# zhanxinrui/HDN

Measured on AMD Instinct MI355X. Metric: frames/sec on 127/255 template/search pairs, higher is better.
Workload: dtype f32; 1 GPU; BASELINE configs[1]: batch=64 synthetic 127/255 pairs per GPU, 256-ch features; HIP kernels only: 1x xcorr 31x31(x)61x61 + 6x xcorr 5x5(x)29x29 + 6x circular xcorr 13x13(x)13x13 + 3x PreShareFeature 127x127 + fused DLT/warp + the 2 L1 scores (one launch); pairs_per_gpu=64, channels=256

## Files before the change

hdn_amd/csrc/xcorr.hip:

```cpp
#include <atomic>

#include "hdn_common.h"
#include "circ13_tables.h"

#include <type_traits>

#include <cstdlib>

#define HDN_ABL_XCORR_0(...) __VA_ARGS__
#define HDN_ABL_XCORR_1(...) __VA_ARGS__
#ifdef HDN_ABLATION
#include "ablation/xcorr.inc"
#endif

namespace hdn {

constexpr int XC_MAX_PROBLEMS = 8;

struct XcorrPtrs {
  const float* x[XC_MAX_PROBLEMS];
  const float* k[XC_MAX_PROBLEMS];
  float* out[XC_MAX_PROBLEMS];
};

namespace prod29 {
constexpr int HX = 29, WX = 29, HK = 5, WK = 5, HO = 25, WO = 25;
constexpr int XPLANE = HX * WX, OPLANE = HO * WO, KPLANE = HK * WK;
constexpr int SX = 37, LPLANE = HX * SX;
constexpr int PPB = 4;
constexpr int UNITS = 5 * WO;
constexpr int XFLOATS = round_up(PPB * LPLANE + 8, 4);
#ifndef PROD29_ALIAS
#define PROD29_ALIAS 0
#endif
#ifndef PROD29_PAD_FLOATS
#define PROD29_PAD_FLOATS 0
#endif
constexpr int LDS_FLOATS = (PROD29_ALIAS ? XFLOATS : XFLOATS + PPB * OPLANE) + PROD29_PAD_FLOATS;
constexpr int N4 = PPB * XPLANE / 4;
constexpr int ITER = cdiv(N4, HDN_BLOCK);
}

__global__ __launch_bounds__(HDN_BLOCK) void xcorr_prod29_kernel(XcorrPtrs P, int planes) {
  using namespace prod29;
  HDN_ABL_XCORR_0()
  __shared__ __attribute__((aligned(16))) float smem[LDS_FLOATS];
  float* sx = smem;
  float* so = PROD29_ALIAS ? smem : smem + XFLOATS;

  const int tid = threadIdx.x;
  const int lane = tid & (HDN_WAVE - 1);
  const int wave = __builtin_amdgcn_readfirstlane(tid >> 6);
  const int prob = blockIdx.y;
  const float* __restrict__ x = P.x[prob];
  const float* __restrict__ k = P.k[prob];
  float* __restrict__ out = P.out[prob];
  const int plane0 = blockIdx.x * PPB;
  const int np = min(PPB, planes - plane0);
  const float* xg = x + size_t(plane0) * XPLANE;

  if (np == PPB && aligned16(xg)) {
    const float4* s4 = reinterpret_cast<const float4*>(xg);
    float4 r[ITER];
#pragma unroll
    for (int q = 0; q < ITER; ++q) r[q] = ld_stream(s4 + min(tid + q * HDN_BLOCK, N4 - 1));
#pragma unroll
    for (int q = 0; q < ITER; ++q) {
      const int i4 = tid + q * HDN_BLOCK;
      if (i4 < N4) {
        const float v[4] = {r[q].x, r[q].y, r[q].z, r[q].w};
        const int e0 = 4 * i4, row0 = e0 / WX, c0 = e0 - row0 * WX;
        if (c0 + 3 < WX) {
          *reinterpret_cast<float4*>(sx + e0 + (SX - WX) * row0) = r[q];
        } else {
#pragma unroll
          for (int t = 0; t < 4; ++t) sx[e0 + t + (SX - WX) * (row0 + (c0 + t >= WX ? 1 : 0))] = v[t];
        }
      }
    }
  } else {
    for (int e = tid; e < np * XPLANE; e += HDN_BLOCK) {
      const int p = e / XPLANE, rem = e - p * XPLANE;
      const int rr = rem / WX, c = rem - rr * WX;
      sx[p * LPLANE + rr * SX + c] = xg[e];
    }
  }
  __syncthreads();

  float held[2][5];
  if (wave < np) {
    const float* __restrict__ kp = k + size_t(plane0 + wave) * KPLANE;
    const float* xs = sx + wave * LPLANE;
    float* os = so + wave * OPLANE;
#pragma unroll
    for (int rd = 0; rd < 2; ++rd) {
      const int unit = rd * HDN_WAVE + lane;
      const int uu = min(unit, UNITS - 1);
      const int b = uu / WO, j = uu - b * WO;
      const float* xc = xs + (5 * b) * SX + j;
      float acc[5] = {0.f, 0.f, 0.f, 0.f, 0.f};
#pragma unroll
      for (int v = 0; v < WK; ++v) {
        float col[9];
#pragma unroll
        for (int r = 0; r < 9; ++r) col[r] = xc[r * SX + v];
#pragma unroll
        for (int u = 0; u < HK; ++u) {
          const float kv = kp[u * WK + v];
#pragma unroll
          for (int t = 0; t < 5; ++t) acc[t] = __builtin_fmaf(col[t + u], kv, acc[t]);
        }
      }
      if constexpr (PROD29_ALIAS) {
#pragma unroll
        for (int t = 0; t < 5; ++t) held[rd][t] = acc[t];
      } else if (unit < UNITS) {
#pragma unroll
        for (int t = 0; t < 5; ++t) os[(5 * b + t) * WO + j] = acc[t];
      }
    }
  }
  __syncthreads();
  if constexpr (PROD29_ALIAS) {
    if (wave < np) {
      float* os = so + wave * OPLANE;
#pragma unroll
      for (int rd = 0; rd < 2; ++rd) {
        const int unit = rd * HDN_WAVE + lane;
        if (unit < UNITS) {
          const int b = unit / WO, j = unit - b * WO;
#pragma unroll
          for (int t = 0; t < 5; ++t) os[(5 * b + t) * WO + j] = held[rd][t];
        }
      }
    }
    __syncthreads();
  }

  float* og = out + size_t(plane0) * OPLANE;
  if (np == PPB && aligned16(og)) copy_l2g_full<PPB * OPLANE>(so, og, tid);
  else copy_l2g(so, og, np * OPLANE, tid);
}

namespace cfg5 {
constexpr int HX = 35, WX = 35, HK = 5, WK = 5, HO = 31, WO = 31;
constexpr int XPLANE = HX * WX, OPLANE = HO * WO, KPLANE = HK * WK;
constexpr int PPB = 4, TH = 8;
constexpr int XFLOATS = round_up(PPB * XPLANE + WX + 4, 4);
constexpr int LDS_FLOATS = XFLOATS + PPB * OPLANE;

typedef const float __attribute__((address_space(4))) cfloat;
template <int V, int M>
__device__ __forceinline__ void strip_pairs(float2v (&Pm)[6], uint32_t a0, uint32_t a1) {
  if constexpr (M < 6) {
    if constexpr (M < 3) Pm[M] = lds_read_pair<(2 * M) * WX + V, (2 * M + 1) * WX + V>(a0);
    else Pm[M] = lds_read_pair<(2 * M - 6) * WX + V, (2 * M - 5) * WX + V>(a1);
    strip_pairs<V, M + 1>(Pm, a0, a1);
  }
}
template <int V>
__device__ __forceinline__ void strip_column(float2v (&accE)[4], float2v (&accO)[5], uint32_t a0, uint32_t a1, const cfloat* kp) {
  float2v Pm[6];
  strip_pairs<V, 0>(Pm, a0, a1);
  lds_wait_all();
#pragma unroll
  for (int m = 0; m < 6; ++m) pin(Pm[m]);
#pragma unroll
  for (int u = 0; u < HK; ++u) {
    const float kv = kp[u * WK + V];
    const float2v kk = {kv, kv};
    if (u % 2 == 0) {
#pragma unroll
      for (int q = 0; q < 4; ++q) accE[q] = __builtin_elementwise_fma(Pm[q + u / 2], kk, accE[q]);
    } else {
#pragma unroll
      for (int q = 0; q < 5; ++q) accO[q] = __builtin_elementwise_fma(Pm[q + u / 2], kk, accO[q]);
    }
  }
}
__device__ __forceinline__ void strip(float (&acc)[TH], const float* x00, const cfloat* kp) {
  float2v accE[4], accO[5];
#pragma unroll
  for (int q = 0; q < 4; ++q) accE[q] = float2v{0.f, 0.f};
#pragma unroll
  for (int q = 0; q < 5; ++q) accO[q] = float2v{0.f, 0.f};
  const uint32_t a0 = lds_addr(x00), a1 = a0 + 6 * WX * 4;
  strip_column<0>(accE, accO, a0, a1, kp);
  strip_column<1>(accE, accO, a0, a1, kp);
  strip_column<2>(accE, accO, a0, a1, kp);
  strip_column<3>(accE, accO, a0, a1, kp);
  strip_column<4>(accE, accO, a0, a1, kp);
#pragma unroll
  for (int q = 0; q < 4; ++q) {
    acc[2 * q] = accE[q].x + accO[q].y;
    acc[2 * q + 1] = accE[q].y + accO[q + 1].x;
  }
}
__device__ __forceinline__ const cfloat* scalar_ptr(const float* p) {
  uint64_t a = reinterpret_cast<uint64_t>(p);
  asm volatile("" : "+s"(a));
  return (const cfloat*)a;
}
}

__global__ __launch_bounds__(HDN_BLOCK) void xcorr_cfg5_kernel(XcorrPtrs P, int planes) {
  using namespace cfg5;
  __shared__ __attribute__((aligned(16))) float smem[XFLOATS];
  float* sx = smem;
  float* so = smem;

  const int tid = threadIdx.x;
  const int lane = tid & (HDN_WAVE - 1);
  const int wave = __builtin_amdgcn_readfirstlane(tid >> 6);
  const int prob = blockIdx.y;
  const float* __restrict__ x = P.x[prob];
  const float* __restrict__ k = P.k[prob];
  float* __restrict__ out = P.out[prob];
  const int plane0 = blockIdx.x * PPB;
  const int np = min(PPB, planes - plane0);
  const float* xg = x + size_t(plane0) * XPLANE;

  if (np == PPB && aligned16(xg)) copy_g2l_full<PPB * XPLANE>(xg, sx, tid);
  else copy_g2l(xg, sx, np * XPLANE, tid);
  if (tid < WX + 4) sx[PPB * XPLANE + tid] = 0.f;
  __syncthreads();

  float accs[2][TH];
  if (wave < np) {
    const cfloat* kp = scalar_ptr(k + size_t(plane0 + wave) * KPLANE);
    const float* xs = sx + wave * XPLANE;
    const int j = min(lane & 31, WO - 1);
#pragma unroll
    for (int rd = 0; rd < 2; ++rd) {
      const int b = 2 * rd + (lane >> 5);
      strip(accs[rd], xs + (TH * b) * WX + j, kp);
    }
  }
  __syncthreads();
  if (wave < np && (lane & 31) < WO) {
    float* os = so + wave * OPLANE;
    const int j = lane & 31;
#pragma unroll
    for (int rd = 0; rd < 2; ++rd) {
      const int b = 2 * rd + (lane >> 5);
#pragma unroll
      for (int t = 0; t < TH; ++t)
        if (TH * b + t < HO) os[(TH * b + t) * WO + j] = accs[rd][t];
    }
  }
  __syncthreads();

  float* og = out + size_t(plane0) * OPLANE;
  if (np == PPB && aligned16(og)) copy_l2g_full<PPB * OPLANE>(so, og, tid);
  else copy_l2g(so, og, np * OPLANE, tid);
}

namespace north {
constexpr int HX = 61, WX = 61, HK = 31, WK = 31, HO = 31, WO = 31;
constexpr int XPLANE = HX * WX;
constexpr int OPLANE = HO * WO;
constexpr int SX = 68;
constexpr int NQUAD = 12;
constexpr int NQ = 15;
constexpr int WINDOW = NQ * HDN_WAVE * 4;
constexpr int GUARD_ROWS_BEFORE = 1, GUARD_ROWS_AFTER = 3;
constexpr int SLOT = (GUARD_ROWS_BEFORE + HX + GUARD_ROWS_AFTER) * SX;
constexpr size_t LDS_BYTES = size_t(4 * SLOT) * sizeof(float);

typedef float f16v __attribute__((ext_vector_type(16)));
typedef float f8v __attribute__((ext_vector_type(8)));
typedef float f4v __attribute__((ext_vector_type(4)));

struct Taps {
  f16v a;
  f8v b;
  f4v c;
  float2v d;
  float e;
  __device__ __forceinline__ float get(int v) const {
    return v < 16 ? a[v] : (v < 24 ? b[v - 16] : (v < 28 ? c[v - 24] : (v < 30 ? d[v - 28] : e)));
  }
};

struct Row {
  f4v Q[NQUAD];
  Taps k;
  __device__ __forceinline__ float2v pair(int n) const { return (n & 1) ? Q[n >> 1].zw : Q[n >> 1].xy; }
};

template <int M>
__device__ __forceinline__ void issue_quads(Row& R, uint32_t a) {
  if constexpr (M < NQUAD) {
    asm volatile("ds_read_b128 %0, %1 offset:%2" : "=v"(R.Q[M]) : "v"(a), "n"(M * 16));
    issue_quads<M + 1>(R, a);
  }
}

__device__ __forceinline__ void load_row(Row& R, uint32_t xaddr, const float* kr) {
  issue_quads<0>(R, xaddr);
  asm volatile(
      "s_nop 4\n\t"
      "s_load_dwordx16 %0, %5, 0x0\n\t"
      "s_load_dwordx8 %1, %5, 0x40\n\t"
      "s_load_dwordx4 %2, %5, 0x60\n\t"
      "s_load_dwordx2 %3, %5, 0x70\n\t"
      "s_load_dword %4, %5, 0x78"
      : "=&s"(R.k.a), "=&s"(R.k.b), "=&s"(R.k.c), "=&s"(R.k.d), "=&s"(R.k.e)
      : "s"(kr));
}

__device__ __forceinline__ void land_row(Row& R) {
  lds_wait_all();
#pragma unroll
  for (int m = 0; m < NQUAD; ++m) asm volatile("" : "+v"(R.Q[m]));
  asm volatile("" : "+s"(R.k.a), "+s"(R.k.b), "+s"(R.k.c), "+s"(R.k.d), "+s"(R.k.e));
  __builtin_amdgcn_sched_barrier(0);
}

__device__ __forceinline__ bool tap_nonzero(float kv) {
  unsigned b;
  asm("s_and_b32 %0, %1, 0x7fffffff" : "=s"(b) : "s"(kv));
  return b != 0u;
}

template <bool LO>
__device__ __forceinline__ void pk_fma_tap(float2v& acc, const float2v& P, const float2v& kpair) {
  if constexpr (LO) asm volatile("v_pk_fma_f32 %0, %1, %2, %0 op_sel_hi:[1,0,1]" : "+v"(acc) : "v"(P), "s"(kpair));
  else asm volatile("v_pk_fma_f32 %0, %1, %2, %0 op_sel:[0,1,0] op_sel_hi:[1,1,1]" : "+v"(acc) : "v"(P), "s"(kpair));
}

template <bool SKIP_ZERO_TAPS>
__device__ __forceinline__ void fma_row(float2v (&accE)[8], float2v (&accO)[8], const Row& R) {
#pragma unroll
  for (int w = 0; w < 16; ++w) {
    const float2v kp = {R.k.get(2 * w), w < 15 ? R.k.get(2 * w + 1) : 0.f};
    if (!SKIP_ZERO_TAPS || tap_nonzero(kp.x)) {
#pragma unroll
      for (int j = 0; j < 8; ++j) pk_fma_tap<true>(accE[j], R.pair(j + w), kp);
    }
    if (w < 15) {
      if (!SKIP_ZERO_TAPS || tap_nonzero(kp.y)) {
#pragma unroll
        for (int j = 0; j < 8; ++j) pk_fma_tap<false>(accO[j], R.pair(j + w), kp);
      }
    }
  }
}

__device__ __forceinline__ void fetch_plane(f4v (&R)[NQ], const float* __restrict__ x, long long first, long long total,
                                            int lane) {
  const bool inside = first >= 0 && first + WINDOW <= total;
  if (inside) {
    const f4v* w = reinterpret_cast<const f4v*>(x + first);
#pragma unroll
    for (int q = 0; q < NQ; ++q) R[q] = w[lane + q * HDN_WAVE];
  } else {
#pragma unroll 1
    for (int q = 0; q < NQ; ++q) {
      const long long f = first + 4 * (lane + q * HDN_WAVE);
      f4v v;
      v.x = (f + 0 >= 0 && f + 0 < total) ? x[f + 0] : 0.f;
      v.y = (f + 1 >= 0 && f + 1 < total) ? x[f + 1] : 0.f;
      v.z = (f + 2 >= 0 && f + 2 < total) ? x[f + 2] : 0.f;
      v.w = (f + 3 >= 0 && f + 3 < total) ? x[f + 3] : 0.f;
#pragma unroll
      for (int qq = 0; qq < NQ; ++qq)
        if (qq == q) R[qq] = v;
    }
  }
}

__device__ __forceinline__ void stash_plane(const f4v (&R)[NQ], uint32_t slot_a, int shift, int lane) {
#pragma unroll
  for (int q = 0; q < NQ; ++q) {
    const int e = 4 * (lane + q * HDN_WAVE) - shift + WX;
    const int row = e / WX, col = e - row * WX;
    const uint32_t a = slot_a + uint32_t(row * SX + col) * 4u;
#pragma unroll
    for (int t = 0; t < 4; ++t) {
      const uint32_t at = a + 4u * t + ((col + t >= WX) ? uint32_t(SX - WX) * 4u : 0u);
      asm volatile("ds_write_b32 %0, %1" : : "v"(at), "v"(R[q][t]));
    }
  }
}
}

template <bool SKIP_ZERO_TAPS>
__device__ __forceinline__ void north_plane(float2v (&accE)[8], float2v (&accO)[8], uint32_t xa, const float* kp) {
  using namespace north;
  Row A, B;
  load_row(A, xa, kp);
  land_row(A);
#pragma unroll 1
  for (int u = 0; u < HK - 1; u += 2) {
    load_row(B, xa + (u + 1) * (SX * 4), kp + (u + 1) * WK);
    __builtin_amdgcn_sched_barrier(0);
    fma_row<SKIP_ZERO_TAPS>(accE, accO, A);
    land_row(B);
    load_row(A, xa + (u + 2) * (SX * 4), kp + (u + 2) * WK);
    __builtin_amdgcn_sched_barrier(0);
    fma_row<SKIP_ZERO_TAPS>(accE, accO, B);
    land_row(A);
  }
  fma_row<SKIP_ZERO_TAPS>(accE, accO, A);
}

template <int MODE>
__global__ __launch_bounds__(HDN_BLOCK, 2) void xcorr_north_kernel(XcorrPtrs P, int planes) {
  using namespace north;
  extern __shared__ __attribute__((aligned(16))) float smem[];

  const int lane = threadIdx.x & (HDN_WAVE - 1);
  const int wave = __builtin_amdgcn_readfirstlane(threadIdx.x >> 6);
  const int prob = blockIdx.y;
  const float* __restrict__ x = P.x[prob];
  const float* __restrict__ k = P.k[prob];
  float* __restrict__ out = P.out[prob];
  const int gw = blockIdx.x * 4 + wave;
  const int nw = gridDim.x * 4;
  if (gw >= planes) return;

  const uint32_t slot_a = lds_addr(smem + wave * SLOT);
  const uint32_t plane_a = slot_a + uint32_t(GUARD_ROWS_BEFORE * SX) * 4u;
  const long long total = (long long)planes * XPLANE;
  const int mis = int((reinterpret_cast<uintptr_t>(x) >> 2) & 3);

  const int i = min(lane & 31, HO - 1);
  const int s = lane >> 5;
  const bool live = (lane & 31) < HO;
  const uint32_t xa = plane_a + uint32_t(i * SX + s * 16) * 4u;

  f4v R[NQ];
  {
    const long long start = (long long)gw * XPLANE;
    fetch_plane(R, x, start - ((start + mis) & 3), total, lane);
  }
#pragma unroll 1
  for (int plane = gw; plane < planes; plane += nw) {
    const long long start = (long long)plane * XPLANE;
    stash_plane(R, slot_a, int((start + mis) & 3), lane);
    if (plane + nw < planes) {
      const long long nstart = (long long)(plane + nw) * XPLANE;
      fetch_plane(R, x, nstart - ((nstart + mis) & 3), total, lane);
    }
    const float* kp = k + size_t(plane) * (HK * WK);
    float2v accE[8], accO[8];
#pragma unroll
    for (int j = 0; j < 8; ++j) accE[j] = accO[j] = float2v{0.f, 0.f};
    north_plane<MODE == 1>(accE, accO, xa, kp);
    const float odd15 = __shfl(accO[0].x, (lane & 31) + 32, HDN_WAVE);
    if (live) {
      float* o = out + size_t(plane) * OPLANE + i * WO + s * 16;
#pragma unroll
      for (int j = 0; j < 8; ++j) {
        o[2 * j] = accE[j].x + accO[j].y;
        if (j < 7) o[2 * j + 1] = accE[j].y + accO[j + 1].x;
      }
      if (s == 0) o[15] = accE[7].y + odd15;
    }
  }
}

namespace circ13f {
constexpr int N = 13, PL = N * N, NF = 7, PPW = 9, WAVES = HDN_BLOCK / 64;
constexpr int XS = 172;
constexpr int TS = 182;
constexpr int REGION = round_up(PPW * TS, 4);
constexpr int WAVE_FLOATS = 2 * REGION;
static_assert(PPW * XS <= REGION, "inputs fit");

typedef float f4e __attribute__((ext_vector_type(4)));
typedef f4e f4u __attribute__((aligned(4)));

__device__ __forceinline__ float2v cmac_conj(float2v acc, float2v k, float2v x) {
  acc = __builtin_elementwise_fma(x, k.xx, acc);
  return __builtin_elementwise_fma(float2v{x.y, -x.x}, k.yy, acc);
}

struct Tw {
  float2v p[6], m[6];
};
__device__ __forceinline__ float2v tw_fwd(const Tw& t, int n) {
  const int k = n % N;
  return k <= 6 ? t.m[k - 1] : t.p[N - k - 1];
}
__device__ __forceinline__ float2v tw_inv(const Tw& t, int n) {
  const int k = n % N;
  return k <= 6 ? t.p[k - 1] : t.m[N - k - 1];
}

__device__ __forceinline__ void dft_col(float2v (&S)[NF], const float* col, const Tw& t) {
  float v[N];
#pragma unroll
  for (int r = 0; r < N; ++r) v[r] = col[r * N];
  float2v sd[7];
  float s0 = v[0];
#pragma unroll
  for (int r = 1; r <= 6; ++r) {
    sd[r] = float2v{v[r] + v[N - r], v[r] - v[N - r]};
    s0 += sd[r].x;
  }
  S[0] = float2v{s0, 0.f};
#pragma unroll
  for (int f = 1; f < NF; ++f) {
    float2v a = float2v{v[0], 0.f};
#pragma unroll
    for (int r = 1; r <= 6; ++r) a = __builtin_elementwise_fma(sd[r], tw_fwd(t, f * r), a);
    S[f] = a;
  }
}

struct Moves {
  static constexpr int WPP = 42, ROUNDS = (PPW * WPP + 63) / 64;
  int g[ROUNDS], l[ROUNDS];
};
__device__ __forceinline__ Moves make_moves(int np, int lane) {
  Moves m;
#pragma unroll
  for (int rd = 0; rd < Moves::ROUNDS; ++rd) {
    const int t = lane + 64 * rd;
    const int q = t / Moves::WPP, w = t - q * Moves::WPP;
    m.g[rd] = q < np ? q * PL + 4 * w : -1;
    m.l[rd] = q * XS + 4 * w;
  }
  return m;
}
struct PlaneRegs {
  f4e v[Moves::ROUNDS];
  float last;
};
__device__ __forceinline__ void planes_load(PlaneRegs& r, const float* __restrict__ g, const Moves& m, int np, int lane) {
#pragma unroll
  for (int rd = 0; rd < Moves::ROUNDS; ++rd) r.v[rd] = *reinterpret_cast<const f4u*>(g + max(m.g[rd], 0));
  r.last = g[min(lane, np - 1) * PL + 168];
}
__device__ __forceinline__ void planes_store(float* lds, const PlaneRegs& r, const Moves& m, int np, int lane) {
#pragma unroll
  for (int rd = 0; rd < Moves::ROUNDS; ++rd)
    if (m.g[rd] >= 0) *reinterpret_cast<f4e*>(lds + m.l[rd]) = r.v[rd];
  if (lane < np) lds[lane * XS + 168] = r.last;
}
__device__ __forceinline__ void planes_out(const float* lds, float* __restrict__ g, const Moves& m, int np, int lane) {
#pragma unroll
  for (int rd = 0; rd < Moves::ROUNDS; ++rd)
    if (m.g[rd] >= 0) *reinterpret_cast<f4u*>(g + m.g[rd]) = *reinterpret_cast<const f4e*>(lds + m.l[rd]);
  if (lane < np) g[lane * PL + 168] = lds[lane * XS + 168];
}
}

__global__ __launch_bounds__(HDN_BLOCK, 3) void xcorr_circ13f_kernel(XcorrPtrs P, int planes, int groups_per_problem, int total_groups) {
  using namespace circ13f;
  HDN_ABL_XCORR_1()
#ifndef CIRC13_PAD_FLOATS
#define CIRC13_PAD_FLOATS 0
#endif
  __shared__ __attribute__((aligned(16))) float smem[WAVES * WAVE_FLOATS + CIRC13_PAD_FLOATS];
  const int lane = threadIdx.x & 63;
  const int wave = __builtin_amdgcn_readfirstlane(threadIdx.x >> 6);
  const int g = blockIdx.x * WAVES + wave;
  if (g >= total_groups) return;
  const int prob = g / groups_per_problem, p0 = (g - prob * groups_per_problem) * PPW, np = min(PPW, planes - p0);
  float* ra = smem + wave * WAVE_FLOATS;
  float* rb = ra + REGION;
  const Moves mv = make_moves(np, lane);
  PlaneRegs rx, rk;
  planes_load(rx, P.x[prob] + size_t(p0) * PL, mv, np, lane);
  planes_load(rk, P.k[prob] + size_t(p0) * PL, mv, np, lane);
  Tw tw;
#pragma unroll
  for (int k = 0; k < 6; ++k) {
    tw.p[k] = float2v{CIRC13_CS[2 * k], CIRC13_CS[2 * k + 1]};
    tw.m[k] = float2v{CIRC13_CS[2 * k], -CIRC13_CS[2 * k + 1]};
  }
  planes_store(ra, rx, mv, np, lane);
  planes_store(rb, rk, mv, np, lane);

  float2v SX[2][NF], SK[2][NF];
  int sq[2], ss[2];
#pragma unroll
  for (int rd = 0; rd < 2; ++rd) {
    const int t = min(lane + 64 * rd, np * N - 1);
    sq[rd] = t / N;
    ss[rd] = t - sq[rd] * N;
    dft_col(SX[rd], ra + sq[rd] * XS + ss[rd], tw);
    dft_col(SK[rd], rb + sq[rd] * XS + ss[rd], tw);
  }
#pragma unroll
  for (int rd = 0; rd < 2; ++rd) {
    if (lane + 64 * rd < np * N) {
      float2v* xp = reinterpret_cast<float2v*>(ra + sq[rd] * TS) + ss[rd];
      float2v* kp = reinterpret_cast<float2v*>(rb + sq[rd] * TS) + ss[rd];
#pragma unroll
      for (int f = 0; f < NF; ++f) {
        xp[f * N] = SX[rd][f];
        kp[f * N] = SK[rd][f];
      }
    }
  }

  {
    const int q = lane / NF, f = lane - q * NF;
    const bool live = q < np;
    const int qa = live ? q : 0;
    const float2v* xp = reinterpret_cast<const float2v*>(ra + qa * TS) + f * N;
    const float2v* kp = reinterpret_cast<const float2v*>(rb + qa * TS) + f * N;
    float2v X[N], K[N];
#pragma unroll
    for (int s = 0; s < N; ++s) {
      X[s] = xp[s];
      K[s] = kp[s];
    }
    float2v PS[7], SS[7];
    PS[0] = K[0];
    SS[0] = K[12];
#pragma unroll
    for (int m = 1; m < 7; ++m) {
      PS[m] = PS[m - 1] + K[m];
      SS[m] = SS[m - 1] + K[12 - m];
    }
    const float zs = f == 0 ? 1.f / 13.f : 2.f / 13.f;
    float2v Z[N];
#pragma unroll
    for (int c = 0; c < N; ++c) {
      float2v z = float2v{0.f, 0.f};
      if (c <= 6) z = cmac_conj(z, PS[6 - c], X[0]);
      if (c >= 6) z = cmac_conj(z, SS[c - 6], X[12]);
#pragma unroll
      for (int j = 0; j < N; ++j) {
        const int s = c + j - 6;
        if (s >= 1 && s <= 11) z = cmac_conj(z, K[j], X[s]);
      }
      Z[c] = z * float2v{zs, zs};
    }
    if (live) {
      float2v* zp = reinterpret_cast<float2v*>(ra + q * TS) + f;
#pragma unroll
      for (int c = 0; c < N; ++c) zp[c * NF] = Z[c];
    }
  }

  float orow[2][N];
#pragma unroll
  for (int rd = 0; rd < 2; ++rd) {
    const float2v* zp = reinterpret_cast<const float2v*>(ra + sq[rd] * TS) + ss[rd] * NF;
    float2v Zf[NF];
#pragma unroll
    for (int f = 0; f < NF; ++f) Zf[f] = zp[f];
    float o0 = Zf[0].x;
#pragma unroll
    for (int f = 1; f < NF; ++f) o0 += Zf[f].x;
    orow[rd][6] = o0;
#pragma unroll
    for (int m = 1; m <= 6; ++m) {
      float2v ab = float2v{0.f, 0.f};
#pragma unroll
      for (int f = 1; f < NF; ++f) ab = __builtin_elementwise_fma(Zf[f], tw_inv(tw, f * m), ab);
      orow[rd][(m + 6) % N] = Zf[0].x + ab.x - ab.y;
      orow[rd][(N - m + 6) % N] = Zf[0].x + ab.x + ab.y;
    }
  }
#pragma unroll
  for (int rd = 0; rd < 2; ++rd) {
    if (lane + 64 * rd < np * N) {
      float* os = rb + sq[rd] * XS + ss[rd];
#pragma unroll
      for (int i = 0; i < N; ++i) os[i * N] = orow[rd][i];
    }
  }
  planes_out(rb, P.out[prob] + size_t(p0) * PL, mv, np, lane);
}

__device__ __forceinline__ int circ_row(int r, int HX) {
  int sr = r - HX / 2;
  return sr < 0 ? sr + HX : (sr >= HX ? sr - HX : sr);
}

template <bool USE_LDS>
__global__ __launch_bounds__(HDN_BLOCK) void xcorr_generic_kernel(XcorrPtrs P, int HX, int WX, int HK, int WK,
                                                                   int circ) {
  extern __shared__ __attribute__((aligned(16))) float smem[];
  const int tid = threadIdx.x;
  const int prob = blockIdx.y;
  const int plane = blockIdx.x;
  const int HP = circ ? HX + 2 * (HX / 2) : HX;
  const int WP = circ ? WX + 2 * (WX / 2) : WX;
  const int HO = HP - HK + 1, WO = WP - WK + 1;
  const float* __restrict__ xg = P.x[prob] + size_t(plane) * HX * WX;
  const float* __restrict__ kg = P.k[prob] + size_t(plane) * HK * WK;
  float* __restrict__ og = P.out[prob] + size_t(plane) * HO * WO;

  if constexpr (USE_LDS) {
    float* xs = smem;
    float* ks = smem + HP * WP;
    for (int idx = tid; idx < HP * WP; idx += HDN_BLOCK) {
      const int r = idx / WP, c = idx - r * WP;
      const int sr = circ ? circ_row(r, HX) : r;
      const int sc = circ ? min(max(c - WX / 2, 0), WX - 1) : c;
      xs[idx] = xg[sr * WX + sc];
    }
    for (int idx = tid; idx < HK * WK; idx += HDN_BLOCK) ks[idx] = kg[idx];
    __syncthreads();
    for (int o = tid; o < HO * WO; o += HDN_BLOCK) {
      const int i = o / WO, j = o - i * WO;
      float acc = 0.f;
      for (int u = 0; u < HK; ++u) {
        const float* xr = xs + (i + u) * WP + j;
        const float* kr = ks + u * WK;
        for (int v = 0; v < WK; ++v) acc = __builtin_fmaf(xr[v], kr[v], acc);
      }
      og[o] = acc;
    }
  } else {
    for (int o = tid; o < HO * WO; o += HDN_BLOCK) {
      const int i = o / WO, j = o - i * WO;
      float acc = 0.f;
      for (int u = 0; u < HK; ++u) {
        const int sr = circ ? circ_row(i + u, HX) : i + u;
        for (int v = 0; v < WK; ++v) {
          const int sc = circ ? min(max(j + v - WX / 2, 0), WX - 1) : j + v;
          acc = __builtin_fmaf(xg[sr * WX + sc], kg[u * WK + v], acc);
        }
      }
      og[o] = acc;
    }
  }
}

static thread_local const char* g_last_variant = "none";

static std::atomic<int> g_north_variant{-1};
static int north_variant() {
  int v = g_north_variant.load(std::memory_order_relaxed);
  if (v >= 0) return v;
  v = HDN_NORTH_FFT_COL;
  const char* e = getenv("HDN_NORTH");
  if (e && e[0] == 'd') v = HDN_NORTH_DIRECT;
  g_north_variant.store(v, std::memory_order_relaxed);
  return v;
}

static int launch_north(const XcorrPtrs& P, int n, int planes, hipStream_t stream) {
  void (*kern)(XcorrPtrs, int) = &xcorr_north_kernel<1>;
  static PerDeviceOnce attr;
  const int dev_ = PerDeviceOnce::device();
  if (!attr.done(dev_)) {
    hipError_t e = hipFuncSetAttribute(reinterpret_cast<const void*>(kern), hipFuncAttributeMaxDynamicSharedMemorySize,
                                       (int)north::LDS_BYTES);
    if (e != hipSuccess) return -(1000 + (int)e);
    attr.set(dev_);
  }
  static const int cap = [] { const char* e = getenv("HDN_NORTH_BLOCKS"); int v = e ? atoi(e) : 0; return v > 0 ? v : 512; }();
  const int per_problem = max(1, min(cdiv(planes, 4), cap / n));
  hipLaunchKernelGGL(kern, dim3(per_problem, n), dim3(HDN_BLOCK), north::LDS_BYTES, stream, P, planes);
  g_last_variant = "north_61x61_31x31";
  return launch_status();
}

int launch_north_fft(const float* x, const float* k, float* out, int planes, int max_blocks, hipStream_t stream, int pair0);
int launch_north_fft4(const float* x, const float* k, float* out, int planes, int max_blocks, hipStream_t stream);
void disarm_north_launch_events();



static int launch_prod29(const XcorrPtrs& P, int n, int planes, hipStream_t stream) {
  hipLaunchKernelGGL(xcorr_prod29_kernel, dim3(cdiv(planes, prod29::PPB), n), dim3(HDN_BLOCK), 0, stream, P, planes);
  g_last_variant = "prod_29x29_5x5";
  return launch_status();
}

static int launch_circ13(const XcorrPtrs& P, int n, int planes, hipStream_t stream) {
  const int gpp = cdiv(planes, circ13f::PPW);
  const long long total = (long long)gpp * n;
  if (total > 0x7fffffffLL) return HDN_E_LIMIT;
  hipLaunchKernelGGL(xcorr_circ13f_kernel, dim3(cdiv((int)total, circ13f::WAVES)), dim3(HDN_BLOCK), 0, stream, P, planes, gpp, (int)total);
  g_last_variant = "circ13";
  return launch_status();
}

static int xcorr_dispatch_(const XcorrPtrs& P, int n, int circular, int B, int C, int Hx, int Wx, int Hk, int Wk, hipStream_t stream);

static int xcorr_dispatch(const XcorrPtrs& P, int n, int circular, int B, int C, int Hx, int Wx, int Hk, int Wk, hipStream_t stream) {
  const int rc = xcorr_dispatch_(P, n, circular, B, C, Hx, Wx, Hk, Wk, stream);
  disarm_north_launch_events();
  return rc;
}

static int xcorr_dispatch_(const XcorrPtrs& P, int n, int circular, int B, int C, int Hx, int Wx, int Hk, int Wk,
                           hipStream_t stream) {
  const long long planes_ll = (long long)B * C;
  if (planes_ll > 0x7fffffffLL / 4) return HDN_E_LIMIT;
  const int planes = (int)planes_ll;
  const int HP = circular ? Hx + 2 * (Hx / 2) : Hx, WP = circular ? Wx + 2 * (Wx / 2) : Wx;
  if ((long long)planes * HP * WP > 0x7fffffffLL) return HDN_E_LIMIT;
  if (!circular) {
    if (Hx == 29 && Wx == 29 && Hk == 5 && Wk == 5) {
      return launch_prod29(P, n, planes, stream);
    }
    if (Hx == 35 && Wx == 35 && Hk == 5 && Wk == 5) {
      hipLaunchKernelGGL(xcorr_cfg5_kernel, dim3(cdiv(planes, cfg5::PPB), n), dim3(HDN_BLOCK), 0, stream, P, planes);
      g_last_variant = "cfg5_35x35_5x5";
      return launch_status();
    }
    if (Hx == 61 && Wx == 61 && Hk == 31 && Wk == 31) {
      const int v = north_variant();
      if (v == HDN_NORTH_FFT_COL) {
        static const int cap = [] { const char* e = getenv("HDN_NORTH_BLOCKS"); int c = e ? atoi(e) : 0; return c > 0 ? c : 1024; }();
        for (int i = 0; i < n; ++i) {
          const int rc = launch_north_fft4(P.x[i], P.k[i], P.out[i], planes, cap, stream);
          if (rc != HDN_OK) return rc;
        }
        g_last_variant = "north_fftc_61x61_31x31";
        return HDN_OK;
      }
      return launch_north(P, n, planes, stream);
    }
  } else {
    if (Hx == 13 && Wx == 13 && Hk == 13 && Wk == 13) return launch_circ13(P, n, planes, stream);
  }
  const size_t lds = (size_t(HP) * WP + size_t(Hk) * Wk) * sizeof(float);
  dim3 grid(planes, n);
  if (lds <= 60 * 1024) {
    hipLaunchKernelGGL(xcorr_generic_kernel<true>, grid, dim3(HDN_BLOCK), lds, stream, P, Hx, Wx, Hk, Wk, circular);
    g_last_variant = "generic_lds";
  } else {
    hipLaunchKernelGGL(xcorr_generic_kernel<false>, grid, dim3(HDN_BLOCK), 0, stream, P, Hx, Wx, Hk, Wk, circular);
    g_last_variant = "generic_l2";
  }
  return launch_status();
}

static int xcorr_check(int B, int C, int Hx, int Wx, int Hk, int Wk, int circular) {
  if (B <= 0 || C <= 0 || Hx <= 0 || Wx <= 0 || Hk <= 0 || Wk <= 0) return HDN_E_SHAPE;
  const int HP = circular ? Hx + 2 * (Hx / 2) : Hx, WP = circular ? Wx + 2 * (Wx / 2) : Wx;
  if (Hk > HP || Wk > WP) return HDN_E_SHAPE;
  if (Hx > 4096 || Wx > 4096) return HDN_E_LIMIT;
  return HDN_OK;
}

}

extern "C" {

const char* hdn_last_xcorr_variant(void) { return hdn::g_last_variant; }

int hdn_xcorr_north_variant(int v) {
  const int prev = hdn::north_variant();
  if (v >= 0) {
    if (v != HDN_NORTH_FFT_COL && v != HDN_NORTH_DIRECT) return HDN_E_LIMIT;
    hdn::g_north_variant.store(v, std::memory_order_relaxed);
  }
  return prev;
}

int hdn_xcorr_depthwise_multi_f32(const float* const* xs, const float* const* ks, float* const* outs, int n,
                                  int circular, int B, int C, int Hx, int Wx, int Hk, int Wk, void* stream) {
  if (!xs || !ks || !outs) return HDN_E_NULL;
  if (n <= 0 || n > hdn::XC_MAX_PROBLEMS) return HDN_E_LIMIT;
  int rc = hdn::xcorr_check(B, C, Hx, Wx, Hk, Wk, circular);
  if (rc) return rc;
  hdn::XcorrPtrs P{};
  for (int i = 0; i < n; ++i) {
    if (!xs[i] || !ks[i] || !outs[i]) return HDN_E_NULL;
    if (outs[i] == xs[i] || outs[i] == ks[i]) return HDN_E_ALIAS;
    P.x[i] = xs[i];
    P.k[i] = ks[i];
    P.out[i] = outs[i];
  }
  return hdn::xcorr_dispatch(P, n, circular, B, C, Hx, Wx, Hk, Wk, static_cast<hipStream_t>(stream));
}

int hdn_xcorr_depthwise_f32(const float* x, const float* k, float* out, int B, int C, int Hx, int Wx, int Hk, int Wk,
                            void* stream) {
  return hdn_xcorr_depthwise_multi_f32(&x, &k, &out, 1, 0, B, C, Hx, Wx, Hk, Wk, stream);
}

int hdn_xcorr_depthwise_circ_f32(const float* x, const float* k, float* out, int B, int C, int Hx, int Wx, int Hk,
                                 int Wk, void* stream) {
  return hdn_xcorr_depthwise_multi_f32(&x, &k, &out, 1, 1, B, C, Hx, Wx, Hk, Wk, stream);
}

}
```

Baseline: 233,700 frames/s.

## Rewrite prod29 xcorr as 13-row register strips with packed FMA and prefetch

The 29x29 by 5x5 correlation kernel now gives each lane one output column and a 13-row strip, with two strips per column overlapping by one row. Input rows are read from LDS as pairs and the next kernel column is double-buffered so loads overlap the packed float2 FMAs. The kernel weights are preloaded into scalar registers through a constant address-space pointer, and the plane is copied unpadded with a zeroed tail row. It also sets a default LDS pad of 1100 floats, presumably to cap occupancy, and raises register pressure in exchange for fewer LDS reads per output.

After: 232,400 frames/s. No clear change (-0.6%).

```diff
diff --git a/hdn_amd/csrc/xcorr.hip b/hdn_amd/csrc/xcorr.hip
--- a/hdn_amd/csrc/xcorr.hip
+++ b/hdn_amd/csrc/xcorr.hip
@@ -23,22 +23,87 @@
   float* out[XC_MAX_PROBLEMS];
 };
 
+typedef const float __attribute__((address_space(4))) cfloat;
+__device__ __forceinline__ const cfloat* scalar_ptr(const float* p) {
+  uint64_t a = reinterpret_cast<uint64_t>(p);
+  asm volatile("" : "+s"(a));
+  return (const cfloat*)a;
+}
+
 namespace prod29 {
 constexpr int HX = 29, WX = 29, HK = 5, WK = 5, HO = 25, WO = 25;
 constexpr int XPLANE = HX * WX, OPLANE = HO * WO, KPLANE = HK * WK;
-constexpr int SX = 37, LPLANE = HX * SX;
-constexpr int PPB = 4;
-constexpr int UNITS = 5 * WO;
-constexpr int XFLOATS = round_up(PPB * LPLANE + 8, 4);
+constexpr int PPB = 4, TH = 13;
+constexpr int ROW1 = HO - TH;
+constexpr int XPAD = round_up(WX + 4, 4);
+constexpr int XFLOATS = PPB * XPLANE + XPAD;
+static_assert(ROW1 + TH + HK <= HX + 1 && (HX + 1) * WX <= XPLANE + XPAD, "a strip reads at most one row beyond its plane");
 #ifndef PROD29_ALIAS
 #define PROD29_ALIAS 0
 #endif
 #ifndef PROD29_PAD_FLOATS
-#define PROD29_PAD_FLOATS 0
+#define PROD29_PAD_FLOATS 1100
 #endif
 constexpr int LDS_FLOATS = (PROD29_ALIAS ? XFLOATS : XFLOATS + PPB * OPLANE) + PROD29_PAD_FLOATS;
-constexpr int N4 = PPB * XPLANE / 4;
-constexpr int ITER = cdiv(N4, HDN_BLOCK);
+
+template <int V, int M>
+__device__ __forceinline__ void strip_pairs(float2v (&Pm)[9], const uint32_t (&a)[3]) {
+  if constexpr (M < 9) {
+    Pm[M] = lds_read_pair<(2 * (M % 3)) * WX + V, (2 * (M % 3) + 1) * WX + V>(a[M / 3]);
+    strip_pairs<V, M + 1>(Pm, a);
+  }
+}
+__device__ __forceinline__ void pin_s(float& v) { asm volatile("" : "+s"(v)); }
+template <int N>
+__device__ __forceinline__ void lds_wait_but() { asm volatile("s_waitcnt lgkmcnt(%0)" ::"n"(N) : "memory"); }
+template <int V>
+__device__ __forceinline__ void strip_column(float2v (&accE)[7], float2v (&accO)[7], float2v (&Pm)[9], float2v (&Pn)[9], const uint32_t (&a)[3],
+                                             const float (&kv)[KPLANE]) {
+  if constexpr (V + 1 < WK) {
+    strip_pairs<V + 1, 0>(Pn, a);
+    lds_wait_but<9>();
+  } else {
+    lds_wait_all();
+  }
+#pragma unroll
+  for (int m = 0; m < 9; ++m) pin(Pm[m]);
+#pragma unroll
+  for (int u = 0; u < HK; ++u) {
+    const float2v kk = {kv[u * WK + V], kv[u * WK + V]};
+    if (u % 2 == 0) {
+#pragma unroll
+      for (int q = 0; q < 7; ++q) accE[q] = __builtin_elementwise_fma(Pm[q + u / 2], kk, accE[q]);
+    } else {
+#pragma unroll
+      for (int q = 0; q < 7; ++q) accO[q] = __builtin_elementwise_fma(Pm[q + u / 2], kk, accO[q]);
+    }
+  }
+#pragma unroll
+  for (int q = 0; q < 7; ++q) pin(accE[q]), pin(accO[q]);
+}
+__device__ __forceinline__ void strip(float (&acc)[TH], const float* x00, const float (&kv)[KPLANE]) {
+  float2v accE[7], accO[7], Pa[9], Pb[9];
+#pragma unroll
+  for (int q = 0; q < 7; ++q) accE[q] = accO[q] = float2v{0.f, 0.f};
+  const uint32_t a0 = lds_addr(x00);
+  const uint32_t a[3] = {a0, a0 + 6 * WX * 4, a0 + 12 * WX * 4};
+  strip_pairs<0, 0>(Pa, a);
+  strip_column<0>(accE, accO, Pa, Pb, a, kv);
+  strip_column<1>(accE, accO, Pb, Pa, a, kv);
+  strip_column<2>(accE, accO, Pa, Pb, a, kv);
+  strip_column<3>(accE, accO, Pb, Pa, a, kv);
+  strip_column<4>(accE, accO, Pa, Pb, a, kv);
+#pragma unroll
+  for (int q = 0; q < 7; ++q) {
+    acc[2 * q] = accE[q].x + accO[q].y;
+    if (q < 6) acc[2 * q + 1] = accE[q].y + accO[q + 1].x;
+  }
+}
+__device__ __forceinline__ void put_strip(float* os, const float (&acc)[TH], int r0, int j) {
+#pragma unroll
+  for (int t = 0; t < TH; ++t)
+    if (t > 0 || r0 == 0) os[(r0 + t) * WO + j] = acc[t];
+}
 }
 
 __global__ __launch_bounds__(HDN_BLOCK) void xcorr_prod29_kernel(XcorrPtrs P, int planes) {
@@ -59,81 +124,28 @@
   const int np = min(PPB, planes - plane0);
   const float* xg = x + size_t(plane0) * XPLANE;
 
-  if (np == PPB && aligned16(xg)) {
-    const float4* s4 = reinterpret_cast<const float4*>(xg);
-    float4 r[ITER];
-#pragma unroll
-    for (int q = 0; q < ITER; ++q) r[q] = ld_stream(s4 + min(tid + q * HDN_BLOCK, N4 - 1));
-#pragma unroll
-    for (int q = 0; q < ITER; ++q) {
-      const int i4 = tid + q * HDN_BLOCK;
-      if (i4 < N4) {
-        const float v[4] = {r[q].x, r[q].y, r[q].z, r[q].w};
-        const int e0 = 4 * i4, row0 = e0 / WX, c0 = e0 - row0 * WX;
-        if (c0 + 3 < WX) {
-          *reinterpret_cast<float4*>(sx + e0 + (SX - WX) * row0) = r[q];
-        } else {
-#pragma unroll
-          for (int t = 0; t < 4; ++t) sx[e0 + t + (SX - WX) * (row0 + (c0 + t >= WX ? 1 : 0))] = v[t];
-        }
-      }
-    }
-  } else {
-    for (int e = tid; e < np * XPLANE; e += HDN_BLOCK) {
-      const int p = e / XPLANE, rem = e - p * XPLANE;
-      const int rr = rem / WX, c = rem - rr * WX;
-      sx[p * LPLANE + rr * SX + c] = xg[e];
-    }
-  }
+  const cfloat* kp = scalar_ptr(k + size_t(min(plane0 + wave, planes - 1)) * KPLANE);
+  float kv[KPLANE];
+#pragma unroll
+  for (int i = 0; i < KPLANE; ++i) kv[i] = kp[i];
+
+  if (np == PPB && aligned16(xg)) copy_g2l_full<PPB * XPLANE>(xg, sx, tid);
+  else copy_g2l(xg, sx, np * XPLANE, tid);
+  if (tid < XPAD) sx[np * XPLANE + tid] = 0.f;
   __syncthreads();
 
-  float held[2][5];
+  const int j = lane & 31, r0 = (lane >> 5) * ROW1;
+  float acc[TH];
+#pragma unroll
+  for (int i = 0; i < KPLANE; ++i) pin_s(kv[i]);
   if (wave < np) {
-    const float* __restrict__ kp = k + size_t(plane0 + wave) * KPLANE;
-    const float* xs = sx + wave * LPLANE;
-    float* os = so + wave * OPLANE;
-#pragma unroll
-    for (int rd = 0; rd < 2; ++rd) {
-      const int unit = rd * HDN_WAVE + lane;
-      const int uu = min(unit, UNITS - 1);
-      const int b = uu / WO, j = uu - b * WO;
-      const float* xc = xs + (5 * b) * SX + j;
-      float acc[5] = {0.f, 0.f, 0.f, 0.f, 0.f};
-#pragma unroll
-      for (int v = 0; v < WK; ++v) {
-        float col[9];
-#pragma unroll
-        for (int r = 0; r < 9; ++r) col[r] = xc[r * SX + v];
-#pragma unroll
-        for (int u = 0; u < HK; ++u) {
-          const float kv = kp[u * WK + v];
-#pragma unroll
-          for (int t = 0; t < 5; ++t) acc[t] = __builtin_fmaf(col[t + u], kv, acc[t]);
-        }
-      }
-      if constexpr (PROD29_ALIAS) {
-#pragma unroll
-        for (int t = 0; t < 5; ++t) held[rd][t] = acc[t];
-      } else if (unit < UNITS) {
-#pragma unroll
-        for (int t = 0; t < 5; ++t) os[(5 * b + t) * WO + j] = acc[t];
-      }
-    }
+    strip(acc, sx + wave * XPLANE + r0 * WX + min(j, WO - 1), kv);
+    if constexpr (!PROD29_ALIAS)
+      if (j < WO) put_strip(so + wave * OPLANE, acc, r0, j);
   }
   __syncthreads();
   if constexpr (PROD29_ALIAS) {
-    if (wave < np) {
-      float* os = so + wave * OPLANE;
-#pragma unroll
-      for (int rd = 0; rd < 2; ++rd) {
-        const int unit = rd * HDN_WAVE + lane;
-        if (unit < UNITS) {
-          const int b = unit / WO, j = unit - b * WO;
-#pragma unroll
-          for (int t = 0; t < 5; ++t) os[(5 * b + t) * WO + j] = held[rd][t];
-        }
-      }
-    }
+    if (wave < np && j < WO) put_strip(so + wave * OPLANE, acc, r0, j);
     __syncthreads();
   }
 
@@ -149,7 +161,6 @@
 constexpr int XFLOATS = round_up(PPB * XPLANE + WX + 4, 4);
 constexpr int LDS_FLOATS = XFLOATS + PPB * OPLANE;
 
-typedef const float __attribute__((address_space(4))) cfloat;
 template <int V, int M>
 __device__ __forceinline__ void strip_pairs(float2v (&Pm)[6], uint32_t a0, uint32_t a1) {
   if constexpr (M < 6) {
@@ -195,11 +206,6 @@
     acc[2 * q] = accE[q].x + accO[q].y;
     acc[2 * q + 1] = accE[q].y + accO[q + 1].x;
   }
-}
-__device__ __forceinline__ const cfloat* scalar_ptr(const float* p) {
-  uint64_t a = reinterpret_cast<uint64_t>(p);
-  asm volatile("" : "+s"(a));
-  return (const cfloat*)a;
 }
 }
 
```
